# zhaodong-liu/GRAM

Hardware: AMD Instinct MI355X
Metric: users/sec @ beam=20 top-20 gen, Beauty T5-base; Recall@5 parity (higher is better)
Workload: dtype f16x3

## Files before the change

gram_amd/_lib.py:

```python
from __future__ import annotations

import ctypes as C
import os

_HERE = os.path.dirname(os.path.abspath(__file__))
LIB_PATH = os.environ.get("GRAM_LIB") or os.path.join(_HERE, "csrc", "libgram_hip.so")

GRAM_MAX_BEAMS = 64
GRAM_MAX_DEC_LEN = 64
GRAM_MAX_PASSAGE_LEN = 128
GRAM_MAX_LONG_PASSAGE_LEN = 512
GRAM_MAX_FUSED_LEN = 4096
GRAM_MAX_LONG_FUSED_LEN = 16384
GRAM_KEY_BITS_LONG_WORDS, GRAM_KEY_BITS_LONG_STRIDE = 512, 528
EPI_BF16, EPI_BF16_RELU, EPI_F32_ADD, EPI_F32, EPI_KV_BANK = range(5)
K_GEMM, K_ENC_ATTN, K_CROSS_ATTN, K_DEC_SELF_ATTN, K_ROWOPS, K_LSE, K_BEAM = range(7)
E_ARG, E_WORKSPACE, E_BEAM, E_NONFINITE = -1, -2, -3, -4
ABI_VERSION = 7
GRAM_TAIL_ENTRY_ROWS = 64
GRAM_TAIL_MAX_STEPS = 16
GRAM_MAX_USER_ITEMS = 4096
ITEMS_EXCLUDE, ITEMS_ALLOW = 0, 1
MAX_PIECES = 2
SPLIT_NPROD = (0, 1, 3)
# ... 155 lines not shown
                                      C.POINTER(Compaction), C.POINTER(UserItems), vp, i64, vp, vp, C.POINTER(i32), vp]),
    "gram_encode_passages": (C.c_int, [vp, vp, vp, C.c_int, C.c_int, vp, i64, vp, vp]),
    "gram_gather_passage_x": (C.c_int, [vp, vp, vp, C.c_int, C.c_int, C.c_int, C.c_int, vp]),
    "gram_live_rows": (C.c_int, [C.POINTER(BeamState), C.POINTER(Trie), C.POINTER(LiveRows), vp]),
    "gram_dec_self_attn_live": (C.c_int, [vp, vp, vp, vp, vp, vp, C.c_int, C.c_int, vp, C.c_int, C.c_int, C.c_int, vp]),
    "gram_cross_attn_decode_live": (C.c_int, [vp, vp, vp, vp, vp, C.c_int, vp, vp, C.c_int, C.c_int, C.c_int, vp]),
    "gram_beam_step_sparse_live": (C.c_int, [C.POINTER(BeamState), C.POINTER(Trie), vp, vp, C.c_int, vp, C.c_int, C.c_int, vp, vp]),
    "gram_gemm_bf16_split": (C.c_int, [vp, vp, vp, C.c_int, C.c_int, C.c_int, C.c_int, C.c_int, C.c_int, C.POINTER(KVBank),
                                       C.POINTER(NormFusion), C.POINTER(Split), vp]),
    "gram_gemm_bf16_lse_split": (C.c_int, [vp, vp, vp, vp, C.c_int, C.c_int, C.c_int, C.c_int, C.c_int, C.POINTER(Split), vp]),
    "gram_embed_ex_split": (C.c_int, [vp, vp, C.c_int, vp, vp, vp, C.c_int, C.c_int, C.c_int, C.c_int, vp]),
    "gram_rmsnorm_bf16_split": (C.c_int, [vp, vp, vp, C.c_int, C.c_int, f32, f32, vp, C.c_int, C.c_int, vp, C.c_int, vp]),
    "gram_enc_self_attn_split": (C.c_int, [vp, vp, vp, vp, C.c_int, C.c_int, C.c_int, C.c_int, i64, vp]),
    "gram_cross_attn_decode_split": (C.c_int, [vp, vp, vp, vp, vp, C.c_int, C.c_int, C.c_int, C.c_int, vp, vp, C.c_int, i64, i64, vp, vp]),
    "gram_enc_self_attn_rows_split": (C.c_int, [vp, vp, vp, vp, vp, C.c_int, C.c_int, C.c_int, C.c_int, i64, vp]),
    "gram_enc_self_attn_long_split": (C.c_int, [vp, vp, vp, vp, C.c_int, C.c_int, C.c_int, C.c_int, i64, vp]),
    "gram_enc_self_attn_long_rows_split": (C.c_int, [vp, vp, vp, vp, vp, C.c_int, C.c_int, C.c_int, C.c_int, i64, vp]),
    "gram_model_set_max_passage_len": (C.c_int, [vp, C.c_int]),
    "gram_mask_key_bits": (C.c_int, [vp, vp, C.c_int, C.c_int, vp]),
    "gram_model_set_max_fused_len": (C.c_int, [vp, C.c_int]),
    "gram_mask_key_bits_long": (C.c_int, [vp, vp, C.c_int, C.c_int, vp]),
    "gram_cross_attn_long_scratch_bytes": (i64, [C.c_int, C.c_int, C.c_int]),
    "gram_cross_attn_long_split": (C.c_int, [vp, vp, vp, vp, vp, C.c_int, C.c_int, C.c_int, C.c_int, vp, vp, C.c_int, i64, i64, vp, vp, vp]),
    "gram_cross_attn_rows_long_split": (C.c_int, [vp, vp, vp, vp, vp, C.c_int, C.c_int, C.c_int, C.c_int, C.c_int, i64, i64, vp, vp, vp, vp]),
    "gram_dec_self_attn_split": (C.c_int, [vp, vp, vp, vp, vp, vp, C.c_int, C.c_int, vp, C.c_int, C.c_int, C.c_int, C.c_int, i64, i64, vp]),
    "gram_dec_self_attn_rows_split": (C.c_int, [vp, vp, vp, vp, vp, vp, vp, C.c_int, C.c_int, vp, C.c_int, C.c_int, C.c_int, C.c_int, i64, i64,
                                                vp]),
    "gram_beam_step_sparse_split": (C.c_int, [C.POINTER(BeamState), C.POINTER(Trie), vp, vp, C.c_int, vp, C.c_int, C.c_int, C.c_int,
                                              vp, C.c_int, vp]),
    "gram_generate": (C.c_int, [vp, vp, vp, C.c_int, C.c_int, C.c_int, C.c_int, C.c_int, C.c_int, f32, C.POINTER(Trie),
                                vp, i64, vp, vp, C.POINTER(i32), vp]),
    "gram_workspace_bytes_tf": (i64, [vp, C.c_int, C.c_int, C.c_int, C.c_int, C.c_int]),
    "gram_teacher_forced": (C.c_int, [vp, vp, vp, C.c_int, C.c_int, C.c_int, C.POINTER(Compaction), vp, vp, C.c_int, C.c_int, vp, i64,
                                      vp, vp, vp, vp]),
    "gram_dec_self_attn_tf_split": (C.c_int, [vp, vp, vp, C.c_int, C.c_int, C.c_int, C.c_int, i64, vp]),
    "gram_cross_attn_rows_split": (C.c_int, [vp, vp, vp, vp, vp, C.c_int, C.c_int, C.c_int, C.c_int, C.c_int, i64, i64, vp, vp, vp]),
    "gram_label_logprob_split": (C.c_int, [vp, vp, vp, C.c_int, vp, vp, C.c_int, C.c_int, C.c_int, C.c_int, vp, vp, vp]),
    "gram_cross_attn_probs_split": (C.c_int, [vp, vp, vp, vp, C.c_int, C.c_int, C.c_int, C.c_int, C.c_int, i64, i64, vp, vp]),
    "gram_xattn_head_sum": (C.c_int, [vp, vp, C.c_int, C.c_int, C.c_int, C.c_int, C.c_int, vp]),
    "gram_xattn_passage_scores": (C.c_int, [vp, vp, vp, C.c_int, C.c_int, C.c_int, C.c_int, f32, vp]),
    "gram_teacher_forced_ex": (C.c_int, [vp, vp, vp, C.c_int, C.c_int, C.c_int, C.POINTER(Compaction), vp, vp, C.c_int, C.c_int, vp, i64,
                                         vp, vp, vp, C.POINTER(XattnOut), vp]),
    "gram_dec_self_attn_tree_split": (C.c_int, [vp, vp, vp, vp, vp, C.c_int, C.c_int, C.c_int, C.c_int, C.c_int, i64, vp]),
    "gram_trie_repeat_tokens": (C.c_int, [vp, vp, C.c_int, C.c_int, vp]),
    "gram_trie_leaf_logprob_split": (C.c_int, [vp, vp, vp, C.c_int, vp, C.POINTER(TrieRows), C.c_int, C.c_int, C.c_int, vp, vp, vp, vp]),
    "gram_workspace_bytes_trie": (i64, [vp, C.c_int, C.c_int, C.c_int, C.c_int]),
    "gram_score_trie": (C.c_int, [vp, vp, vp, C.c_int, C.c_int, C.c_int, C.POINTER(Compaction), C.POINTER(Trie), C.POINTER(TrieRows), vp,
                                  i64, vp, vp, vp]),
    "gram_tail_forest": (C.c_int, [C.POINTER(BeamState), C.POINTER(Trie), C.POINTER(TrieTail), C.POINTER(Forest), C.c_int, vp]),
    "gram_tail_rowpos": (C.c_int, [C.POINTER(BeamState), C.POINTER(Trie), C.POINTER(Forest), vp]),
    "gram_scatter_rows": (C.c_int, [vp, vp, vp, C.c_int, C.c_int, C.c_int, vp]),
    "gram_cross_attn_entries_split": (C.c_int, [vp, vp, vp, vp, vp, C.c_int, C.c_int, C.c_int, C.c_int, vp, vp, C.c_int, i64, i64, vp,
                                                vp]),
    "gram_workspace_bytes_tail": (i64, [vp, C.c_int, C.c_int, C.c_int, C.c_int, C.c_int, C.c_int]),
    "gram_generate_tail": (C.c_int, [vp, vp, vp, C.c_int, C.c_int, C.c_int, C.c_int, C.c_int, C.c_int, f32, C.POINTER(Trie),
                                     C.POINTER(Compaction), C.POINTER(TrieTail), vp, i64, vp, vp, C.POINTER(i32), vp]),
    "gram_debug_set_tail_pass": (C.c_int, [C.c_int]),
    "gram_tail_pass_wanted": (C.c_int, [vp, C.c_int, C.c_int, C.c_int]),
    "gram_debug_set_tail_capacity": (C.c_int, [C.c_int]),
    "gram_debug_set_tail_level_capacity": (C.c_int, [C.c_int]),
    "gram_debug_tail_last": (C.c_int, [C.POINTER(i32)]),
    "gram_debug_workspace_beam_state": (C.c_int, [vp, vp, C.c_int, C.c_int, C.c_int, C.c_int, C.c_int, C.POINTER(BeamState)]),
}

for _old, _new in (("gram_gemm_bf16", "gram_gemm_f16"), ("gram_gemm_bf16_ex", "gram_gemm_f16_ex"), ("gram_gemm_bf16_split", "gram_gemm_f16_split"),
                   ("gram_gemm_bf16_lse", "gram_gemm_f16_lse"), ("gram_gemm_bf16_lse_split", "gram_gemm_f16_lse_split"),
                   ("gram_rmsnorm_bf16", "gram_rmsnorm_f16"), ("gram_rmsnorm_bf16_map", "gram_rmsnorm_f16_map"),
                   ("gram_rmsnorm_bf16_split", "gram_rmsnorm_f16_split")):
    SIGNATURES[_new] = SIGNATURES[_old]

_lib = None


def load() -> C.CDLL:
    global _lib
    if _lib is not None:
        return _lib
    import torch
    if not os.path.exists(LIB_PATH):
        raise ImportError(
            f"{LIB_PATH} not found: the HIP extension is not built (run __graft_entry__.build() or "
            "`make -C gram_amd/csrc`).  gram_amd has no CPU fallback."
        )
    lib = C.CDLL(LIB_PATH)
    for name, (res, args) in SIGNATURES.items():
        fn = getattr(lib, name)
        fn.restype = res
        fn.argtypes = args
    if lib.gram_abi_version() != ABI_VERSION:
        raise ImportError("libgram_hip.so ABI version mismatch")
    _lib = lib
    return lib


class GramHipError(RuntimeError):
    pass


def piece_dtype():
    import torch
    return torch.float16 if load().gram_piece_format() == 1 else torch.bfloat16


def check(code: int, what: str) -> None:
    if code == 0:
        return
# ... 6 lines not shown
```

gram_amd/csrc/generate.hip:

```cpp
#include <stdlib.h>
#include <string.h>
#include <vector>

#include "common.h"
#include "prof.h"

struct gram_model {
  gram_model_desc_t d;
  std::vector<const float*> enc_ln1, enc_ln2, dec_ln1, dec_ln2, dec_ln3;
  std::vector<const void*> enc_wqkv, enc_wo, enc_wi, enc_wo2, dec_wqkv, dec_wo, dec_wq_x, dec_wo_x, dec_wi, dec_wo2;
  std::vector<float> s_enc_wqkv, s_enc_wo, s_enc_wi, s_enc_wo2, s_dec_wqkv, s_dec_wo, s_dec_wq_x, s_dec_wo_x, s_dec_wi, s_dec_wo2;
  float s_wkv = 1.f, s_lm = 1.f;
  const p16 *enc_qkv0 = nullptr, *dec_qkv0 = nullptr;
  int max_L = GRAM_MAX_PASSAGE_LEN;
  int max_S = GRAM_MAX_FUSED_LEN;
  bool long_xattn() const { return max_S > GRAM_MAX_FUSED_LEN; }
};

namespace {

struct Carve {
  char* base;
  int64_t off;
  explicit Carve(void* p) : base((char*)p), off(0) {}
  template <typename T>
  T* take(int64_t n) {
    off = (off + 255) & ~(int64_t)255;
    T* p = base ? reinterpret_cast<T*>(base + off) : nullptr;
    off += n * (int64_t)sizeof(T);
    return p;
  }
};

constexpr int64_t kStreamRowsLimit = GRAM_STREAM_MAX_M_LIMIT;
inline int64_t ss_floats(int64_t rows, int64_t d) {
  const int64_t q = (rows < kStreamRowsLimit ? rows : kStreamRowsLimit) * (d / 16), full = rows * (d / 64);
  return q > full ? q : full;
}
struct Rows {
  float* x;
  p16* h;
  p16* qkv;
  p16* attn;
  p16* qx;
  p16* u;
  float* ss;
  float* rs;
  float* xs[2];
  int64_t ps_qkv, ps_qx;
};
struct Workspace {
  Rows enc, dec;
  p16* bank_k;
  p16* bank_vt;
  p16* kcache;
  p16* vcache;
  float* logits;
  float* lse;
  float* lse_part;
  gram_beam_state_t beam;
  gram_live_rows_t live;
  int32_t* width;
  uint32_t* key_bits;
  float* xa_scratch;
  int32_t* rowmap;
  int64_t bytes;
  gram_forest_t forest;
  Rows tail;
  float *tail_lse, *tail_lse_part;
// ... 371 lines not shown
                                               w.ps_cache, st);
        return gram_dec_self_attn_split(r.qkv, w.kcache + i * cache_layer, w.vcache + i * cache_layer, anc, c.dec_bias_f32, r.attn,
                                        live ? R_cache : R, R, live ? live->rows : nullptr, H, t, Tmax, w.pieces, r.ps_qkv, w.ps_cache, st);
      },
      [&](int i) {
        if (m->long_xattn())
          return gram_cross_attn_long_split(r.qx, w.bank_k + i * bank_layer, w.bank_vt + i * bank_layer, mask, r.attn,
                                            live ? live->n_users : B, K, H, S, live ? live->users : nullptr,
                                            live ? live->rowpos : nullptr, w.pieces, r.ps_qx, w.ps_bank, w.key_bits, w.xa_scratch, st);
        return gram_cross_attn_decode_split(r.qx, w.bank_k + i * bank_layer, w.bank_vt + i * bank_layer, mask, r.attn,
                                            live ? live->n_users : B, K, H, S, live ? live->users : nullptr, live ? live->rowpos : nullptr,
                                            w.pieces, r.ps_qx, w.ps_bank, w.key_bits, st);
      },
      st));
  return lm_head(m, w, R, logits, lse_part, st);
}

int search_step(const gram_model* m, const Workspace& w, const gram_trie_t* trie, int cur_len, int rows_per_user, const int32_t* rowpos,
                const gram_user_items_t* items, void* st) {
  const gram_model_desc_t& c = m->d;
  if (items) {
    if (w.pieces > 1)
      return gram_beam_step_sparse_split_items(&w.beam, trie, w.dec.h, c.lm_head_f32, c.d_model, w.lse, c.vocab, cur_len, rows_per_user,
                                               rowpos, w.pieces, items, st);
    return gram_beam_step_sparse_items(&w.beam, trie, w.dec.h, c.lm_head_bf16, c.d_model, w.lse, c.vocab, cur_len, rows_per_user, rowpos,
                                       items, st);
  }
  if (w.pieces > 1)
    return gram_beam_step_sparse_split(&w.beam, trie, w.dec.h, c.lm_head_f32, c.d_model, w.lse, c.vocab, cur_len, rows_per_user, rowpos,
                                       w.pieces, st);
  if (rowpos) return gram_beam_step_sparse_live(&w.beam, trie, w.dec.h, c.lm_head_bf16, c.d_model, w.lse, c.vocab, cur_len, rowpos, st);
  return gram_beam_step_sparse(&w.beam, trie, w.dec.h, c.lm_head_bf16, c.d_model, w.lse, c.vocab, cur_len, rows_per_user, st);
}

int tail_pass(const gram_model* m, const Workspace& w, const uint8_t* mask, int B, int N, int L, int K, int Tmax, int t0, int n_rows,
              int n_entries, const int32_t* lvl_n, void* st) {
  const gram_model_desc_t& c = m->d;
  const int inner = c.n_heads * 64, H = c.n_heads, S = N * L, R = B * K;
  const size_t bank_layer = (size_t)B * H * S * 64;
  const size_t cache_layer = (size_t)Tmax * R * inner;
  const Rows& r = w.dec;
  const gram_forest_t& f = w.forest;
  const p16* const table = token_table(m, m->dec_qkv0, GRAM_STAGE_DEC_SELF);
  int nlev = f.n_levels, cut = 0;
  for (int g = 0; g < 2; ++g)
    for (int l = 0; l < f.n_levels; ++l)
      if (lvl_n[g * GRAM_TAIL_MAX_STEPS + l] > 0 && t0 + l >= Tmax - 1) cut = 1, nlev = l < nlev ? l : nlev;
  TRY(decoder_layers(
      m, w, f.tokens, n_rows, table != nullptr,
      [&](int i) {
        if (cut) {
          hipError_t e = hipMemsetAsync(r.attn, 0, (size_t)n_rows * inner * w.pieces * sizeof(p16), (hipStream_t)st);
          if (e != hipSuccess) return (int)e;
        }
        for (int g = 0; g < 2; ++g)
          for (int l = 0; l < nlev; ++l) {
            const int n = lvl_n[g * GRAM_TAIL_MAX_STEPS + l];
            if (n < 1) continue;
            const size_t tab = ((size_t)g * f.n_levels + l) * f.cap_rows;
            const int32_t* const rows_l = f.lvl_rows + tab;
            const int32_t* const anc_l = f.lvl_anc + ((size_t)g * f.n_levels + l) * Tmax * R;
            if (i == 0 && table)
              TRY(gram_dec_self_attn_rows_split(table, f.lvl_tokens + tab, w.kcache, w.vcache, anc_l, c.dec_bias_f32, r.qx, R, n, nullptr, H,
                                                t0 + l, Tmax, w.pieces, (int64_t)c.vocab * 3 * inner, w.ps_cache, st));
            else
              TRY(gram_dec_self_attn_rows_split(r.qkv, rows_l, w.kcache + i * cache_layer, w.vcache + i * cache_layer, anc_l, c.dec_bias_f32,
                                                r.qx, R, n, nullptr, H, t0 + l, Tmax, w.pieces, r.ps_qkv, w.ps_cache, st));
            TRY(gram_scatter_rows(r.qx, rows_l, r.attn, n, inner * w.pieces * (int)sizeof(p16), n_rows, st));
          }
        return 0;
      },
      [&](int i) {
        return gram_cross_attn_entries_split(r.qx, w.bank_k + i * bank_layer, w.bank_vt + i * bank_layer, mask, r.attn, n_entries, K, H, S,
                                             f.ent_users, f.ent_rows, w.pieces, r.ps_qx, w.ps_bank, w.key_bits, st);
      },
      st));
  TRY(lm_head(m, w, n_rows, nullptr, w.lse_part, st));
  return gram_lse_combine(w.lse_part, w.lse, n_rows, c.vocab / 64, st);
}
Workspace tail_view(const Workspace& w) {
  Workspace v = w;
  v.dec = w.tail;
  v.lse = w.tail_lse;
  v.lse_part = w.tail_lse_part;
  return v;
}

int g_tail_pass = -1;
int g_tail_cap = 0;
int g_tail_level_cap = 0;
int32_t g_tail_last[4] = {0, 0, 0, 0};
constexpr double kTailMinBankBytes = 256.0 * 1024 * 1024;
bool tail_wanted(const gram_model* m, int B, int N, int L) {
  if (g_tail_pass >= 0) return g_tail_pass != 0;
  const char* e = getenv("GRAM_TAIL_PASS");
  if (e && e[0] == '0') return false;
  if (e && e[0] == '1') return true;
  const int P = m->d.pieces > 1 ? m->d.pieces : 1;
  return 4.0 * B * m->d.n_heads * N * L * 64 * P >= kTailMinBankBytes;
}

}

extern "C" int gram_debug_set_tail_pass(int on) {
  g_tail_pass = on;
  return 0;
// ... 56 lines not shown
  gram_model_desc_t& c = m->d;
  own(m->enc_ln1, c.enc_ln1, c.n_enc_layers);
  own(m->enc_ln2, c.enc_ln2, c.n_enc_layers);
  own(m->enc_wqkv, c.enc_wqkv, c.n_enc_layers);
  own(m->enc_wo, c.enc_wo, c.n_enc_layers);
  own(m->enc_wi, c.enc_wi, c.n_enc_layers);
  own(m->enc_wo2, c.enc_wo2, c.n_enc_layers);
  own(m->dec_ln1, c.dec_ln1, c.n_dec_layers);
  own(m->dec_ln2, c.dec_ln2, c.n_dec_layers);
  own(m->dec_ln3, c.dec_ln3, c.n_dec_layers);
  own(m->dec_wqkv, c.dec_wqkv, c.n_dec_layers);
  own(m->dec_wo, c.dec_wo, c.n_dec_layers);
  own(m->dec_wq_x, c.dec_wq_x, c.n_dec_layers);
  own(m->dec_wo_x, c.dec_wo_x, c.n_dec_layers);
  own(m->dec_wi, c.dec_wi, c.n_dec_layers);
  own(m->dec_wo2, c.dec_wo2, c.n_dec_layers);
  {
    const float* ws = d->w_scales;
    auto take = [&](std::vector<float>& v, int n) {
      v.assign(n, 1.f);
      if (ws) {
        for (int i = 0; i < n; ++i) v[i] = 1.f / ws[i];
        ws += n;
      }
    };
    take(m->s_enc_wqkv, d->n_enc_layers);
    take(m->s_enc_wo, d->n_enc_layers);
    take(m->s_enc_wi, d->n_enc_layers);
    take(m->s_enc_wo2, d->n_enc_layers);
    take(m->s_dec_wqkv, d->n_dec_layers);
    take(m->s_dec_wo, d->n_dec_layers);
    take(m->s_dec_wq_x, d->n_dec_layers);
    take(m->s_dec_wo_x, d->n_dec_layers);
    take(m->s_dec_wi, d->n_dec_layers);
    take(m->s_dec_wo2, d->n_dec_layers);
    if (ws) {
      m->s_wkv = 1.f / ws[0];
      m->s_lm = 1.f / ws[1];
    }
    m->d.w_scales = nullptr;
  }
  return m;
}

extern "C" int gram_model_set_max_passage_len(gram_model_t* m, int Lmax) {
  if (!m || Lmax < GRAM_MAX_PASSAGE_LEN || Lmax > GRAM_MAX_LONG_PASSAGE_LEN || (Lmax & 31)) return GRAM_E_ARG;
  m->max_L = Lmax;
  return 0;
}

extern "C" int gram_model_set_max_fused_len(gram_model_t* m, int Smax) {
  if (!m || Smax < GRAM_MAX_FUSED_LEN || Smax > GRAM_MAX_LONG_FUSED_LEN || (Smax & 31)) return GRAM_E_ARG;
  m->max_S = Smax;
  return 0;
}

extern "C" void gram_model_destroy(gram_model_t* m) {
  if (!m) return;
  delete m;
}

namespace {

struct TableScratch {
  Rows rows;
  int32_t* ids;
  int64_t bytes;
};
TableScratch carve_tables(const gram_model_desc_t& c, void* ws) {
  const int64_t P = c.pieces > 1 ? c.pieces : 1, V = c.vocab, d = c.d_model;
  Carve cv(ws);
  TableScratch t{};
  t.rows.x = cv.take<float>(V * d);
  t.rows.h = cv.take<p16>(P * V * d);
  t.rows.ss = cv.take<float>(ss_floats(V, d));
  t.rows.rs = cv.take<float>(V);
  t.rows.xs[0] = cv.take<float>(V);
  t.rows.xs[1] = cv.take<float>(V);
  t.ids = cv.take<int32_t>(V);
  t.bytes = (cv.off + 255) & ~(int64_t)255;
  return t;
}

int build_table(const gram_model* m, const Workspace& w, const TableScratch& t, const float* gain, const void* wqkv, float s_wqkv,
                p16* table, void* st) {
  const gram_model_desc_t& c = m->d;
  const int V = c.vocab, inner = c.n_heads * 64;
  NormChain nc(m, w, t.rows, V, st);
  TRY(nc.embed(t.ids, 0));
  gram_norm_fusion_t nf;
  const gram_norm_fusion_t* pnf;
  TRY(nc.norm(gain, true, nf, &pnf));
  return linear(w, t.rows.h, wqkv, s_wqkv, table, C_PLANAR, (int64_t)V * 3 * inner, V, 3 * inner, c.d_model, GRAM_EPI_BF16, nullptr, pnf, st);
}

}

extern "C" int64_t gram_token_tables_bytes(const gram_model_t* m) {
  if (!m) return GRAM_E_ARG;
  return m->d.fold_norm ? 2 * token_table_elems(m->d) * (int64_t)sizeof(p16) : 0;
}

extern "C" int64_t gram_token_tables_workspace_bytes(const gram_model_t* m) {
  if (!m) return GRAM_E_ARG;
  return m->d.fold_norm ? carve_tables(m->d, nullptr).bytes : 0;
}
// ... 370 lines not shown
```

gram_amd/model/gram.py:

```python
from __future__ import annotations

import ctypes as C
import math
import os
from typing import Callable, Dict, Optional

import torch
from torch import nn

from .. import _lib
from ..utils.generation_trie import FlatTrie, Trie


class GenerateOutput(dict):

    __getattr__ = dict.get


class ForwardOutput(dict):

    __getattr__ = dict.get

    def to_tuple(self):
        return tuple(v for v in (self.get("loss"), self.get("logits")) if v is not None)
# ... 603 lines not shown
        dec_tab = sd["decoder.block.0.layer.0.SelfAttention.relative_attention_bias.weight"].cpu().float()
        dec_bias = dec_tab[relative_position_bucket(-dist, False, nb, md)].t().contiguous()

        e = "encoder.encoder.block.{}.module.layer"
        dd = "decoder.block.{}.layer"
        ne, nd = self._n_enc, self._n_dec
        wkv_all = torch.cat(
            [torch.cat([sd[dd.format(i) + ".1.EncDecAttention.k.weight"], sd[dd.format(i) + ".1.EncDecAttention.v.weight"]], 0)
             for i in range(nd)], 0)
        inner_ = H * c.d_kv
        kv_row_caps = None
        if "bank_k" in caps or "bank_v" in caps:
            kv_row_caps = torch.tensor([caps.get("bank_k", 99), caps.get("bank_v", 99)]).repeat_interleave(inner_).repeat(nd)
        desc = _lib.ModelDesc(
            vocab=c.vocab_size, d_model=c.d_model, d_ff=c.d_ff, n_heads=H, n_enc_layers=ne, n_dec_layers=nd,
            max_passages=self.max_item_num + 1, tie_word_embeddings=int(bool(getattr(c, "tie_word_embeddings", True))),
            use_position_embedding=int(self.use_position_embedding), fold_norm=int(fold), eps=float(c.layer_norm_epsilon),
            embed_f32=f32(sd["shared.weight"]), lm_head_bf16=b16(sd["lm_head.weight"], "lm_head", no_scale=True),
            pos_emb_f32=f32(sd["position_embedding.weight"]) if self.use_position_embedding else None,
            enc_bias_f32=f32(enc_bias), dec_bias_f32=f32(dec_bias),
            enc_final_ln=f32(sd["encoder.encoder.final_layer_norm.weight"]),
            dec_final_ln=f32(sd["decoder.final_layer_norm.weight"]),
            enc_ln1=ptr_array([f32(sd[e.format(i) + ".0.layer_norm.weight"]) for i in range(ne)]),
            enc_wqkv=ptr_array([qkv(e.format(i) + ".0.SelfAttention", e.format(i) + ".0.layer_norm.weight", "enc_attn") for i in range(ne)]),
            enc_wo=ptr_array([b16(sd[e.format(i) + ".0.SelfAttention.o.weight"], "enc_attn") for i in range(ne)]),
            enc_ln2=ptr_array([f32(sd[e.format(i) + ".1.layer_norm.weight"]) for i in range(ne)]),
            enc_wi=ptr_array([lin(e.format(i) + ".1.DenseReluDense.wi.weight", e.format(i) + ".1.layer_norm.weight", "enc_ffn") for i in range(ne)]),
            enc_wo2=ptr_array([b16(sd[e.format(i) + ".1.DenseReluDense.wo.weight"], "enc_ffn") for i in range(ne)]),
            dec_ln1=ptr_array([f32(sd[dd.format(i) + ".0.layer_norm.weight"]) for i in range(nd)]),
            dec_wqkv=ptr_array([qkv(dd.format(i) + ".0.SelfAttention", dd.format(i) + ".0.layer_norm.weight", "dec_self") for i in range(nd)]),
            dec_wo=ptr_array([b16(sd[dd.format(i) + ".0.SelfAttention.o.weight"], "dec_self") for i in range(nd)]),
            dec_ln2=ptr_array([f32(sd[dd.format(i) + ".1.layer_norm.weight"]) for i in range(nd)]),
            dec_wq_x=ptr_array([lin(dd.format(i) + ".1.EncDecAttention.q.weight", dd.format(i) + ".1.layer_norm.weight", "dec_cross") for i in range(nd)]),
            dec_wo_x=ptr_array([b16(sd[dd.format(i) + ".1.EncDecAttention.o.weight"], "dec_cross") for i in range(nd)]),
            dec_ln3=ptr_array([f32(sd[dd.format(i) + ".2.layer_norm.weight"]) for i in range(nd)]),
            dec_wi=ptr_array([lin(dd.format(i) + ".2.DenseReluDense.wi.weight", dd.format(i) + ".2.layer_norm.weight", "dec_ffn") for i in range(nd)]),
            dec_wo2=ptr_array([b16(sd[dd.format(i) + ".2.DenseReluDense.wo.weight"], "dec_ffn") for i in range(nd)]),
            dec_wkv_x_all=b16(wkv_all, None, kv_row_caps),
            pieces=pieces, lm_head_f32=f32(sd["lm_head.weight"]) if pieces > 1 else None,
        )
        assert len(w_scales) == 4 * ne + 6 * nd + 2
        order = w_scales[1:] + w_scales[:1]
        arr = (C.c_float * len(order))(*order)
        keep.append(arr)
        desc.w_scales = C.cast(arr, C.POINTER(C.c_float))
        handle = lib.gram_model_create(C.byref(desc))
        if not handle:
            raise _lib.GramHipError("gram_model_create rejected the configuration (dims must be multiples of 128, heads <= 16)")
        self._packed = (dev, self._version, handle, keep)
        if self._max_passage_len != _lib.GRAM_MAX_PASSAGE_LEN:
            _lib.check(lib.gram_model_set_max_passage_len(handle, self._max_passage_len), "gram_model_set_max_passage_len")
        if self._max_fused_tokens != _lib.GRAM_MAX_FUSED_LEN:
            _lib.check(lib.gram_model_set_max_fused_len(handle, self._max_fused_tokens), "gram_model_set_max_fused_len")
        self._build_token_tables(handle, keep)
        return handle

    def _build_token_tables(self, handle, keep) -> None:
        lib = _lib.load()
        self._token_tables = None
        need = lib.gram_token_tables_bytes(handle)
        if need <= 0 or os.environ.get("GRAM_TOKEN_TABLES", "1") == "0":
            return
        dev = self._device()
        tables = torch.empty(int(need), dtype=torch.uint8, device=dev)
        scratch = torch.empty(int(lib.gram_token_tables_workspace_bytes(handle)), dtype=torch.uint8, device=dev)
        with torch.cuda.device(dev):
            _lib.check(lib.gram_model_build_token_tables(handle, tables.data_ptr(), tables.numel(), scratch.data_ptr(), scratch.numel(),
                                                         torch.cuda.current_stream(dev).cuda_stream), "gram_model_build_token_tables")
        keep.append(tables)
        self._token_tables = tables

    def _get_workspace(self, handle, B, N, L, K, max_length) -> torch.Tensor:
        lib = _lib.load()
        need = lib.gram_workspace_bytes(handle, B, N, L, K, max_length)
        if need < 0:
            raise _lib.GramHipError(
                f"unsupported problem size B={B} N={N} L={L} K={K} max_length={max_length} "
                f"(N <= max_item_num+1, L <= {self._max_passage_len}, N*L <= {self._max_fused_tokens}, K <= 64, max_length <= {_lib.GRAM_MAX_DEC_LEN}; "
                f"the Trie's fan-out is not limited)"
            )
        return self._ensure_workspace(need)

    def _tail_workspace(self, handle, B, N, L, K, max_length, steps) -> Optional[torch.Tensor]:
        key = (int(handle), B, N, L, K, max_length, steps)
        if key in self._tail_no_fit:
            return None
        dev = self._device()
        need = int(_lib.load().gram_workspace_bytes_tail(handle, B, N, L, K, max_length, steps))
        if need <= 0:
            return None
        cur = self._workspace if self._workspace is not None and self._workspace.device == dev else None
        if cur is not None and cur.numel() >= need:
            return cur
        free, _total = torch.cuda.mem_get_info(dev)
        unused = torch.cuda.memory_reserved(dev) - torch.cuda.memory_allocated(dev)
        room = free + unused + (cur.numel() if cur is not None else 0)
        if need + self._TAIL_FIT_MARGIN <= room:
            try:
                return self._ensure_workspace(need)
            except torch.cuda.OutOfMemoryError:
                pass
        self._tail_no_fit.add(key)
        import warnings
        warnings.warn(f"generate: the tail pass needs a workspace of {need / 2**30:.1f} GiB at B={B}, which does not fit this device "
                      f"next to what it holds; decoding step by step (size the batch with max_users_per_call(..., "
                      f"prefix_allowed_tokens_fn=fn))")
# ... 434 lines not shown
```

include/gram_hip.h:

```cpp
#ifndef GRAM_HIP_H
#define GRAM_HIP_H

#include <stddef.h>
#include <stdint.h>

#ifdef __cplusplus
extern "C" {
#endif

#define GRAM_ABI_VERSION 7

#define GRAM_E_ARG (-1)
#define GRAM_E_WORKSPACE (-2)
#define GRAM_E_BEAM (-3)
#define GRAM_E_NONFINITE (-4)

#define GRAM_MAX_BEAMS 64
#define GRAM_MAX_DEC_LEN 64
#define GRAM_MAX_PASSAGE_LEN 128
#define GRAM_MAX_LONG_PASSAGE_LEN 512
#define GRAM_MAX_FUSED_LEN 4096
#define GRAM_MAX_LONG_FUSED_LEN 16384

enum gram_epilogue {
// ... 264 lines not shown

typedef struct {
  int32_t n_active;
  const int32_t* passage_map;
  const int64_t* ids;
  const uint8_t* mask;
  int32_t n_cached;
  int32_t cache_L;
  const float* cache_x;
  const int32_t* cache_slot;
} gram_compaction_t;
int gram_generate_ex(const gram_model_t* m, const int64_t* input_ids, const uint8_t* mask, int B, int N, int L,
                     int K, int nret, int max_length, float length_penalty, const gram_trie_t* trie_host,
                     const gram_compaction_t* compaction_host, void* workspace, int64_t workspace_bytes,
                     int64_t* sequences, float* scores, int32_t* width_host, void* stream);

int gram_generate_items(const gram_model_t* m, const int64_t* input_ids, const uint8_t* mask, int B, int N, int L, int K, int nret,
                        int max_length, float length_penalty, const gram_trie_t* trie_host, const gram_compaction_t* compaction_host,
                        const gram_user_items_t* items_host, void* workspace, int64_t workspace_bytes, int64_t* sequences,
                        float* scores, int32_t* width_host, void* stream);

#define GRAM_TAIL_MAX_STEPS 16
#define GRAM_TAIL_ENTRY_ROWS 64
typedef struct {
  const int32_t* sub_rows;
  int32_t d_tail;
  int32_t steps;
} gram_trie_tail_t;
typedef struct {
  int32_t* tokens;
  int32_t* pos;
  int32_t* parent;
  int32_t* root;
  int32_t* node;
  int32_t* user_off;
  int32_t* ent_off;
  int32_t* ent_users;
  int32_t* ent_rows;
  int32_t* rowpos;
  int32_t* counts;
  int32_t* slot;
  int32_t* lvl_rows;
  int32_t* lvl_tokens;
  int32_t* lvl_anc;
  int32_t cap_rows, cap_entries, n_levels, pad_;
} gram_forest_t;
int gram_tail_forest(const gram_beam_state_t* st_host, const gram_trie_t* trie_host, const gram_trie_tail_t* tail_host,
                     const gram_forest_t* forest_host, int t, void* stream);
int gram_tail_rowpos(const gram_beam_state_t* st_host, const gram_trie_t* trie_host, const gram_forest_t* forest_host, void* stream);
int gram_scatter_rows(const void* src, const int32_t* rows, void* dst, int n, int row_bytes, int dst_rows, void* stream);
int gram_cross_attn_entries_split(const void* q, const void* k_layer, const void* vt_layer, const uint8_t* mask, void* out,
                                  int n_entries, int K, int H, int S, const int32_t* ent_users, const int32_t* ent_rows, int pieces,
                                  int64_t q_pstride, int64_t bank_pstride, const uint32_t* key_bits, void* stream);
int64_t gram_workspace_bytes_tail(const gram_model_t* m, int B, int N, int L, int K, int max_length, int steps);
int gram_generate_tail(const gram_model_t* m, const int64_t* input_ids, const uint8_t* mask, int B, int N, int L, int K, int nret,
                       int max_length, float length_penalty, const gram_trie_t* trie_host, const gram_compaction_t* compaction_host,
                       const gram_trie_tail_t* tail_host, void* workspace, int64_t workspace_bytes, int64_t* sequences,
                       float* scores, int32_t* width_host, void* stream);

int gram_encode_passages(const gram_model_t* m, const int64_t* ids, const uint8_t* mask, int P, int L,
                         void* workspace, int64_t workspace_bytes, float* x_out, void* stream);
int64_t gram_workspace_encoder_x_offset(const gram_model_t* m, int B, int N, int L, int K, int max_length);
int gram_gather_passage_x(const float* cache_x, const int32_t* slot, float* x, int n, int L, int cache_L, int d,
                          void* stream);


int64_t gram_workspace_bytes_tf(const gram_model_t* m, int B, int N, int L, int C, int T);

int gram_teacher_forced(const gram_model_t* m, const int64_t* input_ids, const uint8_t* mask, int B, int N, int L,
                        const gram_compaction_t* compaction_host, const int32_t* dec_ids, const int32_t* labels, int C, int T,
                        void* workspace, int64_t workspace_bytes, float* logits, float* token_logp, float* seq_logp, void* stream);

int gram_dec_self_attn_tf_split(const void* qkv, const float* bias, void* out, int n_seq, int T, int H, int pieces,
                                int64_t qkv_pstride, void* stream);

int gram_cross_attn_rows_split(const void* q, const void* k_layer, const void* vt_layer, const uint8_t* mask, void* out, int B, int Q,
                               int H, int S, int pieces, int64_t q_pstride, int64_t bank_pstride, const uint32_t* key_bits,
                               int32_t* rowmap, void* stream);
int gram_cross_attn_rows_long_split(const void* q, const void* k_layer, const void* vt_layer, const uint8_t* mask, void* out, int B,
                                    int Q, int H, int S, int pieces, int64_t q_pstride, int64_t bank_pstride, const uint32_t* key_bits,
                                    float* scratch, int32_t* rowmap, void* stream);

int gram_label_logprob_split(const void* hidden, const void* lm_head_bf16, const float* lm_head_f32, int d, const float* lse,
                             const int32_t* labels, int n_seq, int T, int V, int pieces, float* token_logp, float* seq_logp,
                             void* stream);


int gram_cross_attn_probs_split(const void* q, const void* k_layer, const uint8_t* mask, float* probs, int B, int Q, int H, int S,
                                int pieces, int64_t q_pstride, int64_t bank_pstride, const uint32_t* key_bits, void* stream);

int gram_xattn_head_sum(const float* probs, float* acc, int B, int Q, int H, int S, int first, void* stream);

int gram_xattn_passage_scores(const float* acc, const uint8_t* mask, float* scores, int B, int Q, int N, int L, float denom,
                              void* stream);

typedef struct {
  float* probs;
  float* layer_probs;
  float* token_scores;
  float* passage_scores;
} gram_xattn_out_t;

int gram_teacher_forced_ex(const gram_model_t* m, const int64_t* input_ids, const uint8_t* mask, int B, int N, int L,
                           const gram_compaction_t* compaction_host, const int32_t* dec_ids, const int32_t* labels, int C, int T,
                           void* workspace, int64_t workspace_bytes, float* logits, float* token_logp, float* seq_logp,
                           const gram_xattn_out_t* attn_host, void* stream);
// ... 99 lines not shown
```

Measured before the change: 3248.

## Fuse tail-forest decoder self-attention into a single kernel per layer

Adds a forest-aware decoder self-attention kernel that handles every tail level and both groups in one launch. Each row walks its parent chain to gather in-forest keys and values and reads the ancestor cache for earlier steps. This replaces the per-group, per-level loop of row attention plus scatter launches. It is on by default behind an environment switch, which cuts launch count and scatter traffic. In exchange the kernel does per-row pointer chasing through shuffles, and uses custom FMA ordering to keep results matching the old path.

```diff
diff --git a/gram_amd/_lib.py b/gram_amd/_lib.py
--- a/gram_amd/_lib.py
+++ b/gram_amd/_lib.py
@@ -231,6 +231,9 @@
     "gram_scatter_rows": (C.c_int, [vp, vp, vp, C.c_int, C.c_int, C.c_int, vp]),
     "gram_cross_attn_entries_split": (C.c_int, [vp, vp, vp, vp, vp, C.c_int, C.c_int, C.c_int, C.c_int, vp, vp, C.c_int, i64, i64, vp,
                                                 vp]),
+    "gram_dec_self_attn_forest_split": (C.c_int, [vp, vp, C.c_int, vp, vp, vp, C.POINTER(Forest), vp, vp, C.c_int, C.c_int, C.c_int, C.c_int,
+                                                  C.c_int, C.c_int, C.c_int, i64, i64, vp]),
+    "gram_model_set_tail_forest_attn": (C.c_int, [vp, C.c_int]),
     "gram_workspace_bytes_tail": (i64, [vp, C.c_int, C.c_int, C.c_int, C.c_int, C.c_int, C.c_int]),
     "gram_generate_tail": (C.c_int, [vp, vp, vp, C.c_int, C.c_int, C.c_int, C.c_int, C.c_int, C.c_int, f32, C.POINTER(Trie),
                                      C.POINTER(Compaction), C.POINTER(TrieTail), vp, i64, vp, vp, C.POINTER(i32), vp]),
diff --git a/gram_amd/csrc/generate.hip b/gram_amd/csrc/generate.hip
--- a/gram_amd/csrc/generate.hip
+++ b/gram_amd/csrc/generate.hip
@@ -15,6 +15,7 @@
   int max_L = GRAM_MAX_PASSAGE_LEN;
   int max_S = GRAM_MAX_FUSED_LEN;
   bool long_xattn() const { return max_S > GRAM_MAX_FUSED_LEN; }
+  bool tail_forest_attn = false;
 };
 
 namespace {
@@ -492,6 +493,14 @@
         if (cut) {
           hipError_t e = hipMemsetAsync(r.attn, 0, (size_t)n_rows * inner * w.pieces * sizeof(p16), (hipStream_t)st);
           if (e != hipSuccess) return (int)e;
+        }
+        if (m->tail_forest_attn) {
+          if (nlev < 1) return 0;
+          if (i == 0 && table)
+            return gram_dec_self_attn_forest_split(table, f.tokens, c.vocab, w.kcache, w.vcache, w.beam.anc, &f, c.dec_bias_f32, r.attn,
+                                                   n_rows, R, H, t0, nlev, Tmax, w.pieces, (int64_t)c.vocab * 3 * inner, w.ps_cache, st);
+          return gram_dec_self_attn_forest_split(r.qkv, nullptr, 0, w.kcache + i * cache_layer, w.vcache + i * cache_layer, w.beam.anc, &f,
+                                                 c.dec_bias_f32, r.attn, n_rows, R, H, t0, nlev, Tmax, w.pieces, r.ps_qkv, w.ps_cache, st);
         }
         for (int g = 0; g < 2; ++g)
           for (int l = 0; l < nlev; ++l) {
@@ -654,6 +663,12 @@
 extern "C" int gram_model_set_max_fused_len(gram_model_t* m, int Smax) {
   if (!m || Smax < GRAM_MAX_FUSED_LEN || Smax > GRAM_MAX_LONG_FUSED_LEN || (Smax & 31)) return GRAM_E_ARG;
   m->max_S = Smax;
+  return 0;
+}
+
+extern "C" int gram_model_set_tail_forest_attn(gram_model_t* m, int on) {
+  if (!m || (on != 0 && on != 1)) return GRAM_E_ARG;
+  m->tail_forest_attn = on != 0;
   return 0;
 }
 
diff --git a/gram_amd/csrc/self_attn_row.h b/gram_amd/csrc/self_attn_row.h
--- /dev/null
+++ b/gram_amd/csrc/self_attn_row.h
@@ -0,0 +1,77 @@
+#pragma once
+#include "common.h"
+
+namespace gram_sa {
+
+__device__ __forceinline__ float in_f32(float x) {
+  asm volatile("" : "+v"(x));
+  return x;
+}
+
+enum { SA_FMA_ACC = 0, SA_FMA_PV = 1, SA_UNFUSED = 2 };
+constexpr int SA_SELF = 8;
+template <int S>
+constexpr int sa_fuse(int copy, int half) {
+  static_assert(S == 1 || S == 2, "read from the ISA of one and two pieces");
+  if (copy == 3) return SA_UNFUSED;
+  if (half == 1 && (S == 1 || copy == SA_SELF)) return SA_FMA_PV;
+  return SA_FMA_ACC;
+}
+
+struct Row {
+  float m, l, acc[4];
+};
+__device__ __forceinline__ void sa_init(Row& r) {
+  r.m = -INFINITY;
+  r.l = 0.f;
+#pragma unroll
+  for (int e = 0; e < 4; ++e) r.acc[e] = 0.f;
+}
+
+template <int S>
+__device__ __forceinline__ void sa_sum(const p16x4 (&x)[S], float (&o)[4]) {
+#pragma clang fp contract(off)
+#pragma unroll
+  for (int e = 0; e < 4; ++e) o[e] = 0.f;
+#pragma unroll
+  for (int pc = S - 1; pc >= 0; --pc)
+#pragma unroll
+    for (int e = 0; e < 4; ++e) o[e] += (float)x[pc][e];
+}
+
+template <int S, int COPY>
+__device__ __forceinline__ void sa_attend(Row& r, const float (&qf)[4], const float (&kj)[4], const float (&vj)[4], float bias_d) {
+#pragma clang fp contract(off)
+  float s = qf[0] * kj[0] + qf[1] * kj[1] + qf[2] * kj[2] + qf[3] * kj[3];
+  s += __shfl_xor(s, 1, 64);
+  s += __shfl_xor(s, 2, 64);
+  s += __shfl_xor(s, 4, 64);
+  s += __shfl_xor(s, 8, 64);
+  s += bias_d;
+  const float mn = fmaxf(r.m, s);
+  const float alpha = __expf(r.m - mn);
+  const float p = __expf(s - mn);
+  r.m = mn;
+  r.l = fmaf(r.l, alpha, p);
+#pragma unroll
+  for (int e = 0; e < 4; ++e) {
+    const int mode = sa_fuse<S>(COPY, e >> 1);
+    if (mode == SA_FMA_ACC) r.acc[e] = fmaf(r.acc[e], alpha, p * vj[e]);
+    else if (mode == SA_FMA_PV) r.acc[e] = fmaf(vj[e], p, r.acc[e] * alpha);
+    else r.acc[e] = r.acc[e] * alpha + p * vj[e];
+  }
+}
+
+template <int S>
+__device__ __forceinline__ void sa_finish(const Row& r, p16x4 (&o)[S]) {
+#pragma clang fp contract(off)
+  const float inv = 1.f / r.l;
+#pragma unroll
+  for (int e = 0; e < 4; ++e) o[0][e] = (p16)in_f32(r.acc[e] * inv);
+  if constexpr (S == 2) {
+#pragma unroll
+    for (int e = 0; e < 4; ++e) o[1][e] = (p16)in_f32(fmaf(r.acc[e], inv, -(float)o[0][e]));
+  }
+}
+
+}
diff --git a/gram_amd/csrc/tail_attn.hip b/gram_amd/csrc/tail_attn.hip
--- /dev/null
+++ b/gram_amd/csrc/tail_attn.hip
@@ -0,0 +1,139 @@
+#include "common.h"
+#include "prof.h"
+#include "self_attn_row.h"
+
+namespace {
+
+using namespace gram_sa;
+
+__device__ __forceinline__ int clampi(int v, int lo, int hi) { return v < lo ? lo : (v > hi ? hi : v); }
+
+struct ForestAttn {
+  const p16* qkv;
+  const int32_t* qkv_rows;
+  const p16 *kcache, *vcache;
+  const int32_t* anc;
+  const int32_t *pos, *parent, *root;
+  const float* bias;
+  p16* out;
+  long qkv_ps, cache_ps;
+  int qkv_nrows, n_rows, R, H, t0, nlev, nblk;
+};
+
+template <int S, int U>
+__device__ __forceinline__ void forest_step(Row& r, const float (&qf)[4], const p16x4 (&kk)[8][S], const p16x4 (&vv)[8][S], int j, int t,
+                                            const float* __restrict__ bias_h) {
+  if (j < t) {
+    float kj[4], vj[4];
+    sa_sum<S>(kk[U], kj);
+    sa_sum<S>(vv[U], vj);
+    sa_attend<S, U>(r, qf, kj, vj, bias_h[t - j]);
+  }
+}
+
+template <int S>
+__global__ __launch_bounds__(256) void dec_self_attn_forest_kernel(ForestAttn a) {
+  const int per = (a.nblk * a.H + 7) >> 3;
+  const int id = (int)(blockIdx.x & 7) * per + (int)(blockIdx.x >> 3);
+  if (id >= a.nblk * a.H) return;
+  const int blk = id / a.H, h = id - blk * a.H;
+  const int tid = threadIdx.x, l16 = tid & 15, grp = tid >> 4, base = tid & 48;
+  const int i = blk * 16 + grp;
+  if (i >= a.n_rows) return;
+  const int t = a.pos[i], lv = t - a.t0;
+  if (lv < 0 || lv >= a.nlev) return;
+  const int inner = a.H * 64, hoff = h * 64 + 4 * l16;
+  const int rt = clampi(a.root[i], 0, a.R - 1);
+  auto src_row = [&](int row) { return a.qkv_rows ? clampi(a.qkv_rows[row], 0, a.qkv_nrows - 1) : row; };
+  int up = i;
+  for (int s = 0; s <= l16 && s < lv; ++s) up = clampi(a.parent[up], 0, a.n_rows - 1);
+  const int asrc = src_row(up);
+  const int c0 = l16 < a.t0 ? clampi(a.anc[(size_t)l16 * a.R + rt], 0, a.R - 1) : 0;
+  const int c1 = l16 + 16 < a.t0 ? clampi(a.anc[(size_t)(l16 + 16) * a.R + rt], 0, a.R - 1) : 0;
+
+  const p16* self = a.qkv + (size_t)src_row(i) * 3 * inner + hoff;
+  p16x4 q4[S], k4[S], v4[S];
+#pragma unroll
+  for (int pc = 0; pc < S; ++pc) {
+    q4[pc] = *reinterpret_cast<const p16x4*>(self + pc * a.qkv_ps);
+    k4[pc] = *reinterpret_cast<const p16x4*>(self + pc * a.qkv_ps + inner);
+    v4[pc] = *reinterpret_cast<const p16x4*>(self + pc * a.qkv_ps + 2 * inner);
+  }
+  float qf[4], kn[4], vn[4];
+  sa_sum<S>(q4, qf);
+  sa_sum<S>(k4, kn);
+  sa_sum<S>(v4, vn);
+  const float* bias_h = a.bias + h * GRAM_MAX_DEC_LEN;
+  Row r;
+  sa_init(r);
+  constexpr int U = 8;
+  for (int j0 = 0; j0 < t; j0 += U) {
+    p16x4 kk[U][S], vv[U][S];
+#pragma unroll
+    for (int u = 0; u < U; ++u) {
+      const int j = j0 + u;
+      const p16 *kp, *vp;
+      long ps;
+      if (j < a.t0) {
+        const int col = __shfl(j < 16 ? c0 : c1, base + (j & 15), 64);
+        const size_t off = ((size_t)j * a.R + col) * inner + hoff;
+        kp = a.kcache + off;
+        vp = a.vcache + off;
+        ps = a.cache_ps;
+      } else {
+        const int row = __shfl(asrc, base + clampi(t - 1 - j, 0, 15), 64);
+        kp = a.qkv + (size_t)row * 3 * inner + hoff + inner;
+        vp = kp + inner;
+        ps = a.qkv_ps;
+      }
+      const bool live = j < t;
+#pragma unroll
+      for (int pc = 0; pc < S; ++pc) {
+        kk[u][pc] = live ? *reinterpret_cast<const p16x4*>(kp + pc * ps) : (p16x4){(p16)0.f, (p16)0.f, (p16)0.f, (p16)0.f};
+        vv[u][pc] = live ? *reinterpret_cast<const p16x4*>(vp + pc * ps) : (p16x4){(p16)0.f, (p16)0.f, (p16)0.f, (p16)0.f};
+      }
+    }
+    forest_step<S, 0>(r, qf, kk, vv, j0 + 0, t, bias_h);
+    forest_step<S, 1>(r, qf, kk, vv, j0 + 1, t, bias_h);
+    forest_step<S, 2>(r, qf, kk, vv, j0 + 2, t, bias_h);
+    forest_step<S, 3>(r, qf, kk, vv, j0 + 3, t, bias_h);
+    forest_step<S, 4>(r, qf, kk, vv, j0 + 4, t, bias_h);
+    forest_step<S, 5>(r, qf, kk, vv, j0 + 5, t, bias_h);
+    forest_step<S, 6>(r, qf, kk, vv, j0 + 6, t, bias_h);
+    forest_step<S, 7>(r, qf, kk, vv, j0 + 7, t, bias_h);
+  }
+  sa_attend<S, SA_SELF>(r, qf, kn, vn, bias_h[0]);
+  p16x4 o[S];
+  sa_finish<S>(r, o);
+  p16* orow = a.out + (size_t)i * inner * S;
+#pragma unroll
+  for (int pc = 0; pc < S; ++pc) *reinterpret_cast<p16x4*>(orow + (S == 2 ? inter_off(hoff, pc) : hoff)) = o[pc];
+}
+
+}
+
+extern "C" int gram_dec_self_attn_forest_split(const void* qkv, const int32_t* qkv_rows, int qkv_nrows, const void* kcache,
+                                               const void* vcache, const int32_t* anc, const gram_forest_t* forest_host, const float* bias,
+                                               void* out, int n_rows, int R, int H, int t0, int n_levels, int Tmax, int pieces,
+                                               int64_t qkv_pstride, int64_t cache_pstride, void* stream) {
+  const gram_forest_t* f = forest_host;
+  if (!qkv || !f || !f->pos || !f->parent || !f->root || !bias || !out || n_rows < 1 || n_rows > f->cap_rows || R < 1 || H < 1 || H > 16 ||
+      t0 < 0 || n_levels < 1 || n_levels > GRAM_TAIL_MAX_STEPS || Tmax > GRAM_MAX_DEC_LEN || t0 + n_levels > Tmax || pieces < 1 ||
+      pieces > GRAM_MAX_PIECES)
+    return GRAM_E_ARG;
+  if (t0 > 0 && (!kcache || !vcache || !anc)) return GRAM_E_ARG;
+  if (qkv_rows && qkv_nrows < 1) return GRAM_E_ARG;
+  const int64_t src_rows = qkv_rows ? qkv_nrows : n_rows;
+  if (pieces > 1 && (qkv_pstride < src_rows * 3 * H * 64 || (t0 > 0 && cache_pstride < (int64_t)Tmax * R * H * 64))) return GRAM_E_ARG;
+  const int64_t nblk = ((int64_t)n_rows + 15) / 16, wgs = ((nblk * H + 7) / 8) * 8;
+  if (wgs > INT32_MAX / 2) return GRAM_E_ARG;
+  hipStream_t st = (hipStream_t)stream;
+  gram_prof::Scope prof(GRAM_K_DEC_SELF_ATTN, st, 2.0 * 4 * n_rows * H * 64 * pieces);
+  const ForestAttn a{(const p16*)qkv, qkv_rows, (const p16*)kcache, (const p16*)vcache, anc, f->pos, f->parent, f->root, bias,
+                     (p16*)out, (long)qkv_pstride, (long)cache_pstride, qkv_rows ? qkv_nrows : 0, n_rows, R, H, t0, n_levels, (int)nblk};
+  const dim3 grid((unsigned)wgs), block(256);
+  if (pieces == 2) hipLaunchKernelGGL(dec_self_attn_forest_kernel<2>, grid, block, 0, st, a);
+  else hipLaunchKernelGGL(dec_self_attn_forest_kernel<1>, grid, block, 0, st, a);
+  GRAM_CHECK_LAUNCH();
+  return 0;
+}
diff --git a/gram_amd/model/gram.py b/gram_amd/model/gram.py
--- a/gram_amd/model/gram.py
+++ b/gram_amd/model/gram.py
@@ -679,6 +679,8 @@
             _lib.check(lib.gram_model_set_max_passage_len(handle, self._max_passage_len), "gram_model_set_max_passage_len")
         if self._max_fused_tokens != _lib.GRAM_MAX_FUSED_LEN:
             _lib.check(lib.gram_model_set_max_fused_len(handle, self._max_fused_tokens), "gram_model_set_max_fused_len")
+        if os.environ.get("GRAM_TAIL_FOREST_ATTN", "1") != "0":
+            _lib.check(lib.gram_model_set_tail_forest_attn(handle, 1), "gram_model_set_tail_forest_attn")
         self._build_token_tables(handle, keep)
         return handle
 
diff --git a/include/gram_hip.h b/include/gram_hip.h
--- a/include/gram_hip.h
+++ b/include/gram_hip.h
@@ -340,6 +340,11 @@
 int gram_cross_attn_entries_split(const void* q, const void* k_layer, const void* vt_layer, const uint8_t* mask, void* out,
                                   int n_entries, int K, int H, int S, const int32_t* ent_users, const int32_t* ent_rows, int pieces,
                                   int64_t q_pstride, int64_t bank_pstride, const uint32_t* key_bits, void* stream);
+int gram_dec_self_attn_forest_split(const void* qkv, const int32_t* qkv_rows, int qkv_nrows, const void* kcache, const void* vcache,
+                                    const int32_t* anc, const gram_forest_t* forest_host, const float* bias, void* out, int n_rows, int R,
+                                    int H, int t0, int n_levels, int Tmax, int pieces, int64_t qkv_pstride, int64_t cache_pstride,
+                                    void* stream);
+int gram_model_set_tail_forest_attn(gram_model_t* m, int on);
 int64_t gram_workspace_bytes_tail(const gram_model_t* m, int B, int N, int L, int K, int max_length, int steps);
 int gram_generate_tail(const gram_model_t* m, const int64_t* input_ids, const uint8_t* mask, int B, int N, int L, int K, int nret,
                        int max_length, float length_penalty, const gram_trie_t* trie_host, const gram_compaction_t* compaction_host,
```

Measured after the change: 3280, median of 6. Within noise of the previous version (+1.0%).
